# glmanhtu/vit-ed

Hardware: AMD Instinct MI355X
Metric: patch-pairs/sec fwd+bwd, div2k_erosion7_4bin_patch8_64 ViT-ED (higher is better)
Workload: dtype bf16

## Files before the change

vit-ed_amd/csrc/gemm_kernels.h:

```cpp
#pragma once
#include "gemm_epilogue.h"

int gemm_portable(const void* A, int64_t lda, const void* B, int64_t ldb, int b_layout, int dtype, int64_t M, int64_t N,
                  int64_t K, int epilogue, const EpiParams& ep, hipStream_t s);
int gemm_tn_portable(const void* dY, int64_t lddy, const void* X, int64_t ldx, int dtype, int64_t M, int64_t N, int64_t K,
                     int64_t splits, float* out, hipStream_t s);

bool gemm_nt_mfma_supported(const void* A, int64_t lda, const void* B, int64_t ldb, int64_t M, int64_t N, int64_t K,
                            int epilogue, const EpiParams& ep);
int gemm_nt_mfma(const void* A, int64_t lda, const void* B, int64_t ldb, int64_t M, int64_t N, int64_t K, int epilogue,
                 const EpiParams& ep, hipStream_t s);
bool gemm_tn_mfma_supported(const void* dY, int64_t lddy, const void* X, int64_t ldx, int64_t M, int64_t N, int64_t K);
int64_t gemm_tn_mfma_splits(int64_t M, int64_t N, int64_t K);
int gemm_tn_mfma(const void* dY, int64_t lddy, const void* X, int64_t ldx, int64_t M, int64_t N, int64_t K, int64_t splits,
                 float* out, float* bias_out , hipStream_t s);

bool gemm_tn_batch_supported(int count, const int64_t* M, const int64_t* N, const int64_t* K);
void gemm_tn_batch_layout(int count, const int64_t* M, const int64_t* N, const int64_t* K, int64_t* splits, int64_t* slab_stride,
                          int64_t* bias_stride);
int gemm_tn_batch(int count, const void* const* dY, const int64_t* lddy, const void* const* X, const int64_t* ldx, const int64_t* M,
                  const int64_t* N, const int64_t* K, const int* has_bias, float* slabs, float* bias_slabs, hipStream_t s);
int sum_slabs_batch(int count, const float* slabs, int64_t slab_stride, const float* bias_slabs, int64_t bias_stride, int64_t splits,
                    const int64_t* widths, float* const* dW, const int64_t* nbias, float* const* dbias, int accumulate, hipStream_t s);

int sum_rows_f32_single_pass(const float* in, int64_t in_ld, float* out, int64_t batch, int64_t width, hipStream_t s,
                             int accumulate = 0);
int sum_slabs_pair(const float* in_a, int64_t ld_a, float* out_a, int64_t width_a, const float* in_b, int64_t ld_b, float* out_b,
                   int64_t width_b, int64_t batch, hipStream_t s, int accumulate);
```

vit-ed_amd/csrc/gemm_mfma.hip:

```cpp
#include <stdlib.h>

#include <mutex>

#include "gemm_kernels.h"
#include "gemm_nt_epilogue.h"
#include "gemm_lds.h"

template <int BKT, int WM, bool ASM_DMA = false>
__device__ __forceinline__ void nt_stage_load(const bf16* __restrict__ A, int64_t lda, const bf16* __restrict__ B,
                                              int64_t ldb, int64_t m0, int64_t n0, int64_t M, int64_t N, int64_t k0,
                                              char* stage, int wave, int lane) {
    using C = NtCfg<BKT, WM>;
    const int rsub = lane / C::CHUNKS, cp = lane % C::CHUNKS;
#pragma unroll
    for (int i = 0; i < 32 / C::ROWS_PER_DMA; ++i) {
        const int r = wave * 32 + i * C::ROWS_PER_DMA + rsub;
        const int c = cp ^ C::swz(r);
        int64_t gm = m0 + r;
        gm = gm < M ? gm : M - 1;
        const bf16* asrc = A + gm * lda + k0 + c * 8;
        if constexpr (ASM_DMA) glds16_asm(asrc, stage + (wave * 32 + i * C::ROWS_PER_DMA) * C::ROW_BYTES);
        else glds16(asrc, stage + (wave * 32 + i * C::ROWS_PER_DMA) * C::ROW_BYTES);
    }
    constexpr int RB = BN / (2 * WM);
#pragma unroll
    for (int i = 0; i < RB / C::ROWS_PER_DMA; ++i) {
        const int r = wave * RB + i * C::ROWS_PER_DMA + rsub;
        const int c = cp ^ C::swz(r);
        int64_t gn = n0 + r;
        gn = gn < N ? gn : N - 1;
        const bf16* bsrc = B + gn * ldb + k0 + c * 8;
        if constexpr (ASM_DMA) glds16_asm(bsrc, stage + C::A_BYTES + (wave * RB + i * C::ROWS_PER_DMA) * C::ROW_BYTES);
        else glds16(bsrc, stage + C::A_BYTES + (wave * RB + i * C::ROWS_PER_DMA) * C::ROW_BYTES);
    }
}

#ifdef NT_TIMELINE
__device__ unsigned long long nt_timeline[16384 * 4];
extern "C" int vited_debug_timeline(void* dst, int64_t bytes) {
    return hipMemcpyFromSymbol(dst, HIP_SYMBOL(nt_timeline), bytes, 0, hipMemcpyDeviceToHost) == hipSuccess ? 0 : 3;
}
#endif

template <int EPI, int BKT, int WM, int STAGES = 2>
__global__ void __launch_bounds__(128 * WM)
gemm_nt_mfma_kernel(const bf16* __restrict__ A, int64_t lda, const bf16* __restrict__ B, int64_t ldb, int64_t M, int64_t N,
                    int64_t K, int tiles_n, int ntiles, EpiParams ep) {
    extern __shared__ __attribute__((aligned(16))) char smem[];
    const int lane = threadIdx.x & 63;
    const int wave = __builtin_amdgcn_readfirstlane(threadIdx.x >> 6);
    const int wr = wave >> 1, wc = wave & 1;
    const int tile = xcd_remap(blockIdx.x, ntiles);
    const int64_t m0 = (int64_t)(tile / tiles_n) * (64 * WM), n0 = (int64_t)(tile % tiles_n) * BN;

#ifdef NT_STAGGER_US
    if (blockIdx.x < 256 * NT_STAGGER_SLOTS) {
        const int slot = blockIdx.x >> 8;
        for (int i = 0; i < slot * NT_STAGGER_US; ++i) __builtin_amdgcn_s_sleep(32);
    }
#endif
#ifdef NT_TIMELINE
    const unsigned long long tl0 = __builtin_amdgcn_s_memrealtime();
#endif
    f32x4 acc[4][4];
#pragma unroll
    for (int i = 0; i < 4; ++i)
#pragma unroll
        for (int j = 0; j < 4; ++j) acc[i][j] = f32x4{0.f, 0.f, 0.f, 0.f};

    using C = NtCfg<BKT, WM>;
    constexpr bool RING = STAGES >= 3;
    constexpr int PER = 32 / C::ROWS_PER_DMA + (BN / (2 * WM)) / C::ROWS_PER_DMA;
    const int nk = (int)(K / BKT);
    nt_stage_load<BKT, WM, RING>(A, lda, B, ldb, m0, n0, M, N, 0, smem, wave, lane);
    if constexpr (RING) {
#pragma unroll
        for (int pre = 1; pre < STAGES - 1; ++pre)
            if (pre < nk) nt_stage_load<BKT, WM, RING>(A, lda, B, ldb, m0, n0, M, N, (int64_t)pre * BKT, smem + pre * C::STAGE_BYTES, wave, lane);
    }
    const int fr = lane & 15, fq = lane >> 4;
    const int64_t mtile = m0 + wr * 64, ntile = n0 + wc * 64;
    EpiPrefetch<EPI> pf;
    for (int t = 0; t < nk; ++t) {
        if constexpr (RING) {
            const int ahead = nk - 1 - t;
            if (ahead >= STAGES - 2) asm volatile("s_waitcnt vmcnt(%0) lgkmcnt(0)" ::"n"((STAGES - 2) * PER) : "memory");
            else if (ahead == 4 && STAGES > 6) asm volatile("s_waitcnt vmcnt(%0) lgkmcnt(0)" ::"n"(4 * PER) : "memory");
            else if (ahead == 3 && STAGES > 5) asm volatile("s_waitcnt vmcnt(%0) lgkmcnt(0)" ::"n"(3 * PER) : "memory");
            else if (ahead == 2 && STAGES > 4) asm volatile("s_waitcnt vmcnt(%0) lgkmcnt(0)" ::"n"(2 * PER) : "memory");
            else if (ahead == 1 && STAGES > 3) asm volatile("s_waitcnt vmcnt(%0) lgkmcnt(0)" ::"n"(PER) : "memory");
            else asm volatile("s_waitcnt vmcnt(0) lgkmcnt(0)" ::: "memory");
            __builtin_amdgcn_s_barrier();
            asm volatile("" ::: "memory");
        } else {
            asm volatile("s_waitcnt vmcnt(0)" ::: "memory");
            __syncthreads();
        }
        if (t + STAGES - 1 < nk)
            nt_stage_load<BKT, WM, RING>(A, lda, B, ldb, m0, n0, M, N, (int64_t)(t + STAGES - 1) * BKT,
                                         smem + ((t + STAGES - 1) % STAGES) * C::STAGE_BYTES, wave, lane);
        const char* sa = smem + (t % STAGES) * C::STAGE_BYTES;
        const char* sb = sa + C::A_BYTES;
        bf16x8 af[BKT / 32][4], bf_[BKT / 32][4];
#pragma unroll
        for (int kk = 0; kk < BKT / 32; ++kk) {
#pragma unroll
            for (int i = 0; i < 4; ++i) af[kk][i] = *(const bf16x8*)(sa + C::off(wr * 64 + i * 16 + fr, kk * 4 + fq));
#pragma unroll
            for (int j = 0; j < 4; ++j) bf_[kk][j] = *(const bf16x8*)(sb + C::off(wc * 64 + j * 16 + fr, kk * 4 + fq));
        }
        if constexpr (BKT == 64) __builtin_amdgcn_sched_barrier(0);
#pragma unroll
        for (int kk = 0; kk < BKT / 32; ++kk) {
#pragma unroll
            for (int i = 0; i < 4; ++i)
#pragma unroll
                for (int j = 0; j < 4; ++j) {
#ifdef NT_DBG_NO_MFMA
                    asm volatile("" ::"v"(af[kk][i]), "v"(bf_[kk][j]));
#else
                    acc[i][j] = __builtin_amdgcn_mfma_f32_16x16x32_bf16(af[kk][i], bf_[kk][j], acc[i][j], 0, 0, 0);
#endif
                }
        }
    }
#ifdef NT_DBG_NO_EPI
#pragma unroll
    for (int i = 0; i < 4; ++i)
#pragma unroll
        for (int j = 0; j < 4; ++j) asm volatile("" ::"v"(acc[i][j]));
    return;
#endif
#ifdef NT_TIMELINE
    const unsigned long long tl1 = __builtin_amdgcn_s_memrealtime();
#endif
    epilogue_prefetch_bias<EPI>(ep, pf, ntile, N, lane);
    epilogue_prefetch_subtile<EPI>(ep, pf, 0, mtile, ntile, M, N, lane);
    __syncthreads();
    float* sc = (float*)(smem + wave * SCRATCH_BYTES);
#pragma unroll
    for (int i = 0; i < 4; ++i) {
        if (i + 1 < 4) epilogue_prefetch_subtile<EPI>(ep, pf, i + 1, mtile, ntile, M, N, lane);
#pragma unroll
        for (int j = 0; j < 4; ++j)
#pragma unroll
            for (int e = 0; e < 4; ++e) sc[(fq * 4 + e) * SCRATCH_LD + j * 16 + fr] = acc[i][j][e];
        asm volatile("" ::: "memory");
        epilogue_subtile<EPI>(ep, pf, sc, i, mtile, ntile, M, N, lane);
        asm volatile("" ::: "memory");
    }
#ifdef NT_TIMELINE
    if (threadIdx.x == 0 && blockIdx.x < 16384) {
        asm volatile("s_waitcnt vmcnt(0)" ::: "memory");
        const unsigned long long tl2 = __builtin_amdgcn_s_memrealtime();
        const unsigned hw = __builtin_amdgcn_s_getreg(63492), xcc = __builtin_amdgcn_s_getreg(6164);
        nt_timeline[blockIdx.x * 4 + 0] = tl0;
        nt_timeline[blockIdx.x * 4 + 1] = tl1;
        nt_timeline[blockIdx.x * 4 + 2] = tl2;
        nt_timeline[blockIdx.x * 4 + 3] = ((unsigned long long)xcc << 32) | hw;
    }
#endif
}

bool gemm_nt_mfma_supported(const void* A, int64_t lda, const void* B, int64_t ldb, int64_t M, int64_t N, int64_t K,
                            int epilogue, const EpiParams& ep) {
    auto al16 = [](const void* p) { return ((uintptr_t)p & 15) == 0; };
    if (K % 64 || N % 16 || lda % 8 || ldb % 8 || ep.ldo % 8) return false;
    if (!al16(A) || !al16(B) || !al16(ep.out)) return false;
    if (ep.bias && !al16(ep.bias)) return false;
    if ((epilogue == VITED_EPI_GELU || epilogue == VITED_EPI_GELU_GRAD) && !al16(ep.out2)) return false;
    if ((epilogue == VITED_EPI_MUL_GELU_GRAD || epilogue == VITED_EPI_MUL) && !al16(ep.aux)) return false;
    if (epilogue == VITED_EPI_RESIDUAL && !al16(ep.residual)) return false;
    if (ceil_div64(M, 128) * ceil_div64(N, BN) > (1 << 30)) return false;
    if (M >= ((int64_t)1 << 31) || ep.rows_per_batch >= ((int64_t)1 << 31)) return false;
    return true;
}

template <int EPI, int BKT, int WM, int STAGES = 2>
static int launch_nt(const bf16* a, int64_t lda, const bf16* b, int64_t ldb, int64_t M, int64_t N, int64_t K, const EpiParams& ep,
                      hipStream_t s) {
    using C = NtCfg<BKT, WM>;
    const int tiles_n = (int)ceil_div64(N, BN);
    const int ntiles = (int)ceil_div64(M, C::BM) * tiles_n;
    auto kernel = gemm_nt_mfma_kernel<EPI, BKT, WM, STAGES>;
    constexpr int LDS = STAGES * C::STAGE_BYTES;
    if (LDS > 65536) {
        static std::once_flag once;
        static hipError_t status = hipSuccess;
        std::call_once(once, [&] { status = hipFuncSetAttribute((const void*)kernel, hipFuncAttributeMaxDynamicSharedMemorySize, LDS); });
        if (status != hipSuccess) return VITED_ERR_LAUNCH;
    }
    hipLaunchKernelGGL(kernel, dim3(ntiles), dim3(128 * WM), LDS, s, a, lda, b, ldb, M, N, K, tiles_n, ntiles, ep);
    return VITED_OK;
}

template <int EPI>
static int dispatch_nt(const bf16* a, int64_t lda, const bf16* b, int64_t ldb, int64_t M, int64_t N, int64_t K, const EpiParams& ep,
                       hipStream_t s) {
    bool shallow = K <= 512 && N >= 768;
    constexpr bool tall_epi = EPI == VITED_EPI_STORE || EPI == VITED_EPI_MUL || EPI == VITED_EPI_GELU_GRAD;
    bool tall = tall_epi && shallow && N >= 768 && M >= 8192;
#ifdef VITED_TUNING
    static const int force_bk = getenv("VITED_NT_BK") ? atoi(getenv("VITED_NT_BK")) : 0;
    static const int force_wm = getenv("VITED_NT_WM") ? atoi(getenv("VITED_NT_WM")) : 0;
    static const int force_st = getenv("VITED_NT_STAGES") ? atoi(getenv("VITED_NT_STAGES")) : 0;
    if (force_bk) shallow = force_bk == 32;
    if (force_wm) tall = force_wm == 4;
    if (force_st == 3) {
        if (shallow && tall) return launch_nt<EPI, 32, 4, 3>(a, lda, b, ldb, M, N, K, ep, s);
        if (shallow) return launch_nt<EPI, 32, 2, 3>(a, lda, b, ldb, M, N, K, ep, s);
        if (tall) return launch_nt<EPI, 64, 4, 3>(a, lda, b, ldb, M, N, K, ep, s);
        return launch_nt<EPI, 64, 2, 3>(a, lda, b, ldb, M, N, K, ep, s);
    }
#endif
    if (shallow && tall && EPI == VITED_EPI_STORE) return launch_nt<EPI, 32, 4, 3>(a, lda, b, ldb, M, N, K, ep, s);
    if (shallow && tall) return launch_nt<EPI, 32, 4>(a, lda, b, ldb, M, N, K, ep, s);
    if (shallow) return launch_nt<EPI, 32, 2>(a, lda, b, ldb, M, N, K, ep, s);
    if (tall) return launch_nt<EPI, 64, 4>(a, lda, b, ldb, M, N, K, ep, s);
    return launch_nt<EPI, 64, 2>(a, lda, b, ldb, M, N, K, ep, s);
}

int gemm_nt_mfma(const void* A, int64_t lda, const void* B, int64_t ldb, int64_t M, int64_t N, int64_t K, int epilogue,
                 const EpiParams& ep, hipStream_t s) {
    const bf16* a = (const bf16*)A;
    const bf16* b = (const bf16*)B;
    int rc;
    switch (epilogue) {
        case VITED_EPI_STORE: rc = dispatch_nt<VITED_EPI_STORE>(a, lda, b, ldb, M, N, K, ep, s); break;
        case VITED_EPI_GELU: rc = dispatch_nt<VITED_EPI_GELU>(a, lda, b, ldb, M, N, K, ep, s); break;
        case VITED_EPI_RESIDUAL: rc = dispatch_nt<VITED_EPI_RESIDUAL>(a, lda, b, ldb, M, N, K, ep, s); break;
        case VITED_EPI_MUL_GELU_GRAD: rc = dispatch_nt<VITED_EPI_MUL_GELU_GRAD>(a, lda, b, ldb, M, N, K, ep, s); break;
        case VITED_EPI_STORE_F32: rc = dispatch_nt<VITED_EPI_STORE_F32>(a, lda, b, ldb, M, N, K, ep, s); break;
        case VITED_EPI_MUL: rc = dispatch_nt<VITED_EPI_MUL>(a, lda, b, ldb, M, N, K, ep, s); break;
        case VITED_EPI_GELU_GRAD: rc = dispatch_nt<VITED_EPI_GELU_GRAD>(a, lda, b, ldb, M, N, K, ep, s); break;
        default: return VITED_ERR_BAD_ARG;
    }
    return rc != VITED_OK ? rc : vited_check_launch();
}

#ifndef TN_FORCE_TM
#define TN_FORCE_TM 0
#define TN_FORCE_STAGES 0
#endif

__device__ __forceinline__ int tn_f(int r) { return ((r & 3) << 2) | ((r >> 2) & 3); }

__device__ __forceinline__ bf16x4 tr_read(const char* p) {
    return __builtin_amdgcn_ds_read_tr16_b64_v4bf16((__attribute__((address_space(3))) bf16x4*)p);
}

template <int TM, bool ASM_DMA>
__device__ __forceinline__ void tn_stage_load(const bf16* __restrict__ dY, int64_t lddy, const bf16* __restrict__ X,
                                              int64_t ldx, int64_t mrow0, int64_t mlast, int64_t n0, int64_t N,
                                              int64_t kc0, int64_t K, char* stage, int wave, int lane) {
    constexpr int T_TILE_BYTES = TM * 128 * 2;
    const int rsub = lane >> 4, cp = lane & 15;
#pragma unroll
    for (int i = 0; i < TM / 16; ++i) {
        const int r = wave * (TM / 4) + i * 4 + rsub;
        const int ch = cp ^ tn_f(r);
        int64_t gm = mrow0 + r;
        gm = gm <= mlast ? gm : mlast;
        int64_t cn = n0 + ch * 8;
        cn = cn <= N - 8 ? cn : N - 8;
        int64_t ck = kc0 + ch * 8;
        ck = ck <= K - 8 ? ck : K - 8;
        if constexpr (ASM_DMA) {
            glds16_asm(dY + gm * lddy + cn, stage + (wave * (TM / 4) + i * 4) * 256);
            glds16_asm(X + gm * ldx + ck, stage + T_TILE_BYTES + (wave * (TM / 4) + i * 4) * 256);
        } else {
            glds16(dY + gm * lddy + cn, stage + (wave * (TM / 4) + i * 4) * 256);
            glds16(X + gm * ldx + ck, stage + T_TILE_BYTES + (wave * (TM / 4) + i * 4) * 256);
        }
    }
}

template <bool BIAS, int TM, int TN_STAGES>
__global__ void __launch_bounds__(256) __attribute__((amdgpu_waves_per_eu(3)))
gemm_tn_mfma_kernel(const bf16* __restrict__ dY, int64_t lddy, const bf16* __restrict__ X, int64_t ldx, int64_t M, int64_t N,
                    int64_t K, int64_t rows_per_split, int tiles_k, float* __restrict__ out, float* __restrict__ bias_out) {
    extern __shared__ __attribute__((aligned(16))) char smem[];
    constexpr int T_TILE_BYTES = TM * 128 * 2, T_STAGE_BYTES = 2 * T_TILE_BYTES;
    constexpr bool RING = TN_STAGES >= 3;
    const int lane = threadIdx.x & 63;
    const int wave = __builtin_amdgcn_readfirstlane(threadIdx.x >> 6);
    const int wr = wave >> 1, wc = wave & 1;
    const int ntile = gridDim.x;
    const int lin = xcd_remap(blockIdx.x + blockIdx.y * ntile, ntile * gridDim.y);
    const int split = lin / ntile, tile_id = lin - split * ntile;
    const int64_t n0 = (int64_t)(tile_id / tiles_k) * 128, kc0 = (int64_t)(tile_id % tiles_k) * 128;
    const int64_t mb = (int64_t)split * rows_per_split;
    int64_t me = mb + rows_per_split;
    me = me < M ? me : M;

    f32x4 acc[4][4];
    float bsum[4] = {0.f, 0.f, 0.f, 0.f};
#pragma unroll
    for (int i = 0; i < 4; ++i) {
#pragma unroll
        for (int j = 0; j < 4; ++j) acc[i][j] = f32x4{0.f, 0.f, 0.f, 0.f};
    }

    const int nsteps = me > mb ? (int)((me - mb + TM - 1) / TM) : 0;
    if (nsteps > 0) tn_stage_load<TM, RING>(dY, lddy, X, ldx, mb, me - 1, n0, N, kc0, K, smem, wave, lane);
    if constexpr (RING) {
#pragma unroll
        for (int pre = 1; pre < TN_STAGES - 1; ++pre)
            if (nsteps > pre) tn_stage_load<TM, RING>(dY, lddy, X, ldx, mb + pre * TM, me - 1, n0, N, kc0, K, smem + pre * T_STAGE_BYTES, wave, lane);
    }
    const int g = lane >> 4, q = (lane & 15) >> 2, p = lane & 3;
    for (int t = 0; t < nsteps; ++t) {
        if constexpr (RING) {
            constexpr int PER = 2 * (TM / 16);
            const int ahead = nsteps - 1 - t;
            if (ahead >= TN_STAGES - 2) asm volatile("s_waitcnt vmcnt(%0)" ::"n"((TN_STAGES - 2) * PER) : "memory");
            else if (ahead == 2 && TN_STAGES > 4) asm volatile("s_waitcnt vmcnt(%0)" ::"n"(2 * PER) : "memory");
            else if (ahead == 1 && TN_STAGES > 3) asm volatile("s_waitcnt vmcnt(%0)" ::"n"(PER) : "memory");
            else asm volatile("s_waitcnt vmcnt(0)" ::: "memory");
        } else {
            asm volatile("s_waitcnt vmcnt(0)" ::: "memory");
        }
        char* st = smem + (t % TN_STAGES) * T_STAGE_BYTES;
        const int64_t mrow0 = mb + (int64_t)t * TM;
        if (mrow0 + TM > me) {
            const int rsub = lane >> 4, cp = lane & 15;
#pragma unroll
            for (int i = 0; i < TM / 16; ++i) {
                const int r = wave * (TM / 4) + i * 4 + rsub;
                if (mrow0 + r >= me) {
                    *(f32x4*)(st + r * 256 + cp * 16) = f32x4{0.f, 0.f, 0.f, 0.f};
                    *(f32x4*)(st + T_TILE_BYTES + r * 256 + cp * 16) = f32x4{0.f, 0.f, 0.f, 0.f};
                }
            }
        }
        if constexpr (RING) {
            asm volatile("s_waitcnt lgkmcnt(0)" ::: "memory");
            __builtin_amdgcn_s_barrier();
            asm volatile("" ::: "memory");
        } else {
            __syncthreads();
        }
        if (t + TN_STAGES - 1 < nsteps)
            tn_stage_load<TM, RING>(dY, lddy, X, ldx, mrow0 + (TN_STAGES - 1) * TM, me - 1, n0, N, kc0, K,
                                    smem + ((t + TN_STAGES - 1) % TN_STAGES) * T_STAGE_BYTES, wave, lane);
        const char* sy = st;
        const char* sx = st + T_TILE_BYTES;
#ifdef TN_DBG_DMA_ONLY
        continue;
#endif
#pragma unroll
        for (int ms = 0; ms < TM / 32; ++ms) {
            bf16x8 af[4], bf_[4];
            const int r_lo = ms * 32 + 8 * g + q, r_hi = r_lo + 4;
            const int f_lo = tn_f(r_lo), f_hi = tn_f(r_hi);
#pragma unroll
            for (int i = 0; i < 4; ++i) {
                const int ch = ((wr * 64 + i * 16) >> 3) + (p >> 1);
                const bf16x4 lo = tr_read(sy + r_lo * 256 + ((ch ^ f_lo) << 4) + 8 * (p & 1));
                const bf16x4 hi = tr_read(sy + r_hi * 256 + ((ch ^ f_hi) << 4) + 8 * (p & 1));
                af[i] = bf16x8{lo[0], lo[1], lo[2], lo[3], hi[0], hi[1], hi[2], hi[3]};
            }
#pragma unroll
            for (int j = 0; j < 4; ++j) {
                const int ch = ((wc * 64 + j * 16) >> 3) + (p >> 1);
                const bf16x4 lo = tr_read(sx + r_lo * 256 + ((ch ^ f_lo) << 4) + 8 * (p & 1));
                const bf16x4 hi = tr_read(sx + r_hi * 256 + ((ch ^ f_hi) << 4) + 8 * (p & 1));
                bf_[j] = bf16x8{lo[0], lo[1], lo[2], lo[3], hi[0], hi[1], hi[2], hi[3]};
            }
#pragma unroll
            for (int i = 0; i < 4; ++i)
#pragma unroll
                for (int j = 0; j < 4; ++j) {
#ifdef TN_DBG_NO_MFMA
                    asm volatile("" ::"v"(af[i]), "v"(bf_[j]));
#else
                    acc[i][j] = __builtin_amdgcn_mfma_f32_16x16x32_bf16(bf_[j], af[i], acc[i][j], 0, 0, 0);
#endif
                }
            if (BIAS && kc0 == 0) {
                typedef __attribute__((ext_vector_type(2))) __bf16 bf16x2_t;
                const bf16x2_t one2 = {(__bf16)1.0f, (__bf16)1.0f};
#pragma unroll
                for (int i = 0; i < 4; ++i) {
#pragma unroll
                    for (int e = 0; e < 4; ++e)
                        bsum[i] = __builtin_amdgcn_fdot2_f32_bf16(bf16x2_t{af[i][2 * e], af[i][2 * e + 1]}, one2, bsum[i], false);
                }
            }
        }
    }
    float* o = out + (int64_t)split * N * K;
    const int fr = lane & 15, fq = lane >> 4;
#pragma unroll
    for (int i = 0; i < 4; ++i) {
#pragma unroll
        for (int j = 0; j < 4; ++j) {
            const int64_t n = n0 + wr * 64 + i * 16 + fr;
            const int64_t k = kc0 + wc * 64 + j * 16 + fq * 4;
#ifdef TN_DBG_NO_STORE
            asm volatile("" ::"v"(acc[i][j]));
#else
            if (n < N && k < K) *(f32x4*)(o + n * K + k) = acc[i][j];
#endif
        }
    }
    if constexpr (BIAS) {
        if (kc0 == 0 && wc == 0) {
            float* bo = bias_out + (int64_t)split * N;
#pragma unroll
            for (int i = 0; i < 4; ++i) {
                float v = bsum[i];
                v += __shfl_xor(v, 16);
                v += __shfl_xor(v, 32);
                const int64_t n = n0 + wr * 64 + i * 16 + fr;
                if (fq == 0 && n < N) bo[n] = v;
            }
        }
    }
}

#define TW_STAGES 4
#define TW_PANEL_BYTES (32 * 256)
#define TW_STAGE_BYTES (4 * TW_PANEL_BYTES)
#define TW_PER 4

__device__ __forceinline__ void tw_stage_issue(const bf16* const (&src)[4], char* stage, int panel, int rbase) {
#pragma unroll
    for (int i = 0; i < 4; ++i) glds16_asm(src[i], stage + panel * TW_PANEL_BYTES + (rbase + i * 4) * 256);
}

struct TwFrags {
    bf16x8 a[4], b[6];
};

__device__ __forceinline__ void tw_read_frags(TwFrags& f, const char* st, const int (&ya_lo)[4], const int (&ya_hi)[4],
                                              const int (&xb_lo)[6], const int (&xb_hi)[6]) {
#pragma unroll
    for (int i = 0; i < 4; ++i) {
        const bf16x4 lo = tr_read(st + ya_lo[i]);
        const bf16x4 hi = tr_read(st + ya_hi[i]);
        f.a[i] = bf16x8{lo[0], lo[1], lo[2], lo[3], hi[0], hi[1], hi[2], hi[3]};
    }
#pragma unroll
    for (int j = 0; j < 6; ++j) {
        const bf16x4 lo = tr_read(st + xb_lo[j]);
        const bf16x4 hi = tr_read(st + xb_hi[j]);
        f.b[j] = bf16x8{lo[0], lo[1], lo[2], lo[3], hi[0], hi[1], hi[2], hi[3]};
    }
}

#define TW_MAX_PROBLEMS 40
struct TwProblem {
    const bf16* dY;
    const bf16* X;
    int64_t lddy, ldx, M, rows_per_split;
    int64_t slab_off, bias_off;
    int N, K, tiles_k, tile0;
    int has_bias, pad_;
};
struct TwBatch {
    TwProblem p[TW_MAX_PROBLEMS];
    int64_t slab_stride, bias_stride;
    int count, total_tiles;
};

template <bool BIAS>
__global__ void __launch_bounds__(512)
gemm_tn_wide_kernel(const TwBatch batch, float* __restrict__ out_base, float* __restrict__ bias_base) {
    extern __shared__ __attribute__((aligned(16))) char smem[];
    const int lane = threadIdx.x & 63;
    const int wave = __builtin_amdgcn_readfirstlane(threadIdx.x >> 6);
    const int wr = wave >> 2, wc = wave & 3;
    const int ntile = batch.total_tiles;
    const int lin = xcd_remap(blockIdx.x + blockIdx.y * ntile, ntile * gridDim.y);
    const int split = lin / ntile;
    int tile_id = lin - split * ntile;
    int pi = 0;
    for (int i = 1; i < batch.count; ++i)
        if (batch.p[i].tile0 <= tile_id) pi = i;
    const TwProblem& pr = batch.p[pi];
    tile_id -= pr.tile0;
    const bf16* __restrict__ dY = pr.dY;
    const bf16* __restrict__ X = pr.X;
    const int64_t lddy = pr.lddy, ldx = pr.ldx, M = pr.M, N = pr.N, K = pr.K, rows_per_split = pr.rows_per_split;
    const int tiles_k = pr.tiles_k;
    const bool with_bias = BIAS && pr.has_bias;
    float* __restrict__ out = out_base + pr.slab_off;
    float* __restrict__ bias_out = bias_base + pr.bias_off;
    const int64_t n0 = (int64_t)(tile_id / tiles_k) * 128, kc0 = (int64_t)(tile_id % tiles_k) * 384;
    const int64_t mb = (int64_t)split * rows_per_split;
    int64_t me = mb + rows_per_split;
    me = me < M ? me : M;
    const int nsteps = me > mb ? (int)((me - mb + 31) / 32) : 0;

    f32x4 acc[4][6];
    float bsum[4] = {0.f, 0.f, 0.f, 0.f};
#pragma unroll
    for (int i = 0; i < 4; ++i) {
#pragma unroll
        for (int j = 0; j < 6; ++j) acc[i][j] = f32x4{0.f, 0.f, 0.f, 0.f};
    }

    const int panel = wave >> 1, rbase = (wave & 1) * 16;
    const int rsub = lane >> 4, cp = lane & 15;
    const bf16* const pbase = panel == 0 ? dY : X;
    const int64_t ld = panel == 0 ? lddy : ldx;
    const int64_t col0 = panel == 0 ? n0 : kc0 + (panel - 1) * 128;
    const int64_t colmax = panel == 0 ? N - 8 : col0 + 120;
    int64_t coff[4];
#pragma unroll
    for (int i = 0; i < 4; ++i) {
        int64_t c = col0 + ((cp ^ tn_f(rbase + i * 4 + rsub)) << 3);
        coff[i] = c <= colmax ? c : colmax;
    }
    const bf16* p0[4];
#pragma unroll
    for (int i = 0; i < 4; ++i) p0[i] = pbase + (mb + rbase + i * 4 + rsub) * ld + coff[i];
    const int64_t stage_stride = 32 * ld;
    const int rows_here = (int)(me - mb);
    auto issue = [&](int stage_idx) {
        char* dst = smem + (stage_idx & (TW_STAGES - 1)) * TW_STAGE_BYTES;
        if ((stage_idx + 1) * 32 <= rows_here) {
            const int64_t adv = (int64_t)stage_idx * stage_stride;
            const bf16* src[4];
#pragma unroll
            for (int i = 0; i < 4; ++i) src[i] = p0[i] + adv;
            tw_stage_issue(src, dst, panel, rbase);
        } else {
            const bf16* src[4];
#pragma unroll
            for (int i = 0; i < 4; ++i) {
                int r = stage_idx * 32 + rbase + i * 4 + rsub;
                r = r < rows_here ? r : rows_here - 1;
                src[i] = pbase + (mb + r) * ld + coff[i];
            }
            tw_stage_issue(src, dst, panel, rbase);
        }
    };
    auto wait_landed = [&](int idx) {
        const int later = (nsteps - 1 < idx + TW_STAGES - 2 ? nsteps - 1 : idx + TW_STAGES - 2) - idx;
        if (later >= 3 && TW_STAGES > 4) asm volatile("s_waitcnt vmcnt(%0)" ::"n"(3 * TW_PER) : "memory");
        else if (later >= 2) asm volatile("s_waitcnt vmcnt(%0)" ::"n"(2 * TW_PER) : "memory");
        else if (later == 1) asm volatile("s_waitcnt vmcnt(%0)" ::"n"(TW_PER) : "memory");
        else asm volatile("s_waitcnt vmcnt(0)" ::: "memory");
        if ((idx + 1) * 32 > rows_here) {
            char* st = smem + (idx & (TW_STAGES - 1)) * TW_STAGE_BYTES;
#pragma unroll
            for (int i = 0; i < 4; ++i) {
                const int r = rbase + i * 4 + rsub;
                if (idx * 32 + r >= rows_here) *(f32x4*)(st + panel * TW_PANEL_BYTES + r * 256 + cp * 16) = f32x4{0.f, 0.f, 0.f, 0.f};
            }
        }
    };

    const int g = lane >> 4, q = (lane & 15) >> 2, p = lane & 3;
    const int r_lo = 8 * g + q, r_hi = r_lo + 4;
    const int f_lo = tn_f(r_lo), f_hi = tn_f(r_hi);
    int ya_lo[4], ya_hi[4], xb_lo[6], xb_hi[6];
#pragma unroll
    for (int i = 0; i < 4; ++i) {
        const int ch = ((wr * 64 + i * 16) >> 3) + (p >> 1);
        ya_lo[i] = r_lo * 256 + ((ch ^ f_lo) << 4) + 8 * (p & 1);
        ya_hi[i] = r_hi * 256 + ((ch ^ f_hi) << 4) + 8 * (p & 1);
    }
#pragma unroll
    for (int j = 0; j < 6; ++j) {
        const int col = wc * 96 + j * 16;
        const int ch = ((col & 127) >> 3) + (p >> 1);
        const int base = (1 + (col >> 7)) * TW_PANEL_BYTES;
        xb_lo[j] = base + r_lo * 256 + ((ch ^ f_lo) << 4) + 8 * (p & 1);
        xb_hi[j] = base + r_hi * 256 + ((ch ^ f_hi) << 4) + 8 * (p & 1);
    }

    auto slot_l = [&](int t, TwFrags& f) {
#ifndef TW_DBG_NO_READS
        tw_read_frags(f, smem + (t & (TW_STAGES - 1)) * TW_STAGE_BYTES, ya_lo, ya_hi, xb_lo, xb_hi);
#endif
#ifndef TW_DBG_NO_DMA
        if (t + TW_STAGES - 1 < nsteps) issue(t + TW_STAGES - 1);
#endif
        __builtin_amdgcn_s_waitcnt(0xc07f);
    };
    auto slot_m = [&](const TwFrags& cur) {
        __builtin_amdgcn_s_setprio(1);
#pragma unroll
        for (int j = 0; j < 6; ++j)
#pragma unroll
            for (int i = 0; i < 4; ++i) {
#ifdef TW_DBG_NO_MFMA
                asm volatile("" ::"v"(cur.b[j]), "v"(cur.a[i]));
#else
                acc[i][j] = __builtin_amdgcn_mfma_f32_16x16x32_bf16(cur.b[j], cur.a[i], acc[i][j], 0, 0, 0);
#endif
            }
        __builtin_amdgcn_s_setprio(0);
        if (with_bias && kc0 == 0) {
            typedef __attribute__((ext_vector_type(2))) __bf16 bf16x2_t;
            const bf16x2_t one2 = {(__bf16)1.0f, (__bf16)1.0f};
#pragma unroll
            for (int i = 0; i < 4; ++i) {
#pragma unroll
                for (int e = 0; e < 4; ++e)
                    bsum[i] = __builtin_amdgcn_fdot2_f32_bf16(bf16x2_t{cur.a[i][2 * e], cur.a[i][2 * e + 1]}, one2, bsum[i], false);
            }
        }
    };
    auto barrier = [&]() {
        __builtin_amdgcn_s_barrier();
        asm volatile("" ::: "memory");
    };
    auto certify_barrier = [&](int idx) {
        __builtin_amdgcn_sched_barrier(0);
        if (idx < nsteps) {
            wait_landed(idx);
            asm volatile("s_waitcnt lgkmcnt(0)" ::: "memory");
        }
        barrier();
    };

    if (nsteps > 0) {
#pragma unroll
        for (int pre = 0; pre < TW_STAGES - 1; ++pre)
            if (nsteps > pre) issue(pre);
        certify_barrier(0);
        TwFrags f;
        if (wr == 0) {
            for (int t = 0; t < nsteps; ++t) {
                slot_l(t, f);
                barrier();
                slot_m(f);
                certify_barrier(t + 1);
            }
            barrier();
        } else {
            barrier();
            for (int t = 0; t < nsteps; ++t) {
                slot_l(t, f);
                certify_barrier(t + 1);
                slot_m(f);
                barrier();
            }
        }
    }

    float* o = out + (int64_t)split * batch.slab_stride;
    const int fr = lane & 15, fq = lane >> 4;
#pragma unroll
    for (int i = 0; i < 4; ++i) {
        const int64_t n = n0 + wr * 64 + i * 16 + fr;
#pragma unroll
        for (int j = 0; j < 6; ++j) {
            const int64_t k = kc0 + wc * 96 + j * 16 + fq * 4;
            if (n < N) *(f32x4*)(o + n * K + k) = acc[i][j];
        }
    }
    if constexpr (BIAS) {
        if (with_bias && kc0 == 0 && wc == 0) {
            float* bo = bias_out + (int64_t)split * batch.bias_stride;
#pragma unroll
            for (int i = 0; i < 4; ++i) {
                float v = bsum[i];
                v += __shfl_xor(v, 16);
                v += __shfl_xor(v, 32);
                const int64_t n = n0 + wr * 64 + i * 16 + fr;
                if (fq == 0 && n < N) bo[n] = v;
            }
        }
    }
}

bool gemm_tn_mfma_supported(const void* dY, int64_t lddy, const void* X, int64_t ldx, int64_t M, int64_t N, int64_t K) {
    auto al16 = [](const void* p) { return ((uintptr_t)p & 15) == 0; };
    return N % 8 == 0 && K % 8 == 0 && N >= 8 && K >= 8 && lddy % 8 == 0 && ldx % 8 == 0 && al16(dY) && al16(X) && M >= 1;
}

static inline bool tn_use_ring(int64_t M, int64_t N, int64_t K) {
    if (TN_FORCE_TM) return TN_FORCE_STAGES >= 3;
#ifdef VITED_TUNING
    static const char* env = getenv("VITED_TN_RING");
    if (env) return atoi(env) != 0;
#endif
    return N * K >= 1536 * 384 && M >= 16384;
}

static inline bool tn_use_wide(int64_t M, int64_t N, int64_t K) {
    if (TN_FORCE_TM) return false;
    if (K % 384 != 0) return false;
#ifdef VITED_TUNING
    static const char* env = getenv("VITED_TN_WIDE");
    if (env) return atoi(env) != 0;
#endif
    return M >= 4096;
}

int64_t gemm_tn_mfma_splits(int64_t M, int64_t N, int64_t K) {
    if (tn_use_wide(M, N, K)) {
        const int64_t tiles = ceil_div64(N, 128) * (K / 384);
        int64_t slots = 256;
#ifdef VITED_TUNING
        static const int64_t slots_env = getenv("VITED_TN_WIDE_SLOTS") ? atoi(getenv("VITED_TN_WIDE_SLOTS")) : 0;
        if (slots_env) slots = slots_env;
#endif
        int64_t s = slots / tiles;
        const int64_t max_s = ceil_div64(M, 256);
        if (s > max_s) s = max_s;
        if (s < 1) s = 1;
        const int64_t rps = ceil_div64(ceil_div64(M, s), 32) * 32;
        return ceil_div64(M, rps);
    }
    const bool ring = tn_use_ring(M, N, K);
    const int tm = TN_FORCE_TM ? TN_FORCE_TM : (ring ? 32 : 64);
    const int64_t tiles = ceil_div64(N, 128) * ceil_div64(K, 128);
    int64_t slots = tm == 64 ? 512 : 768;
#ifdef VITED_TUNING
    static const int64_t slots_env = getenv("VITED_TN_SLOTS") ? atoi(getenv("VITED_TN_SLOTS")) : 0;
    if (slots_env) slots = slots_env;
#endif
    int64_t s = slots / tiles;
    const int64_t max_s = ceil_div64(M, 512);
    if (s > max_s) s = max_s;
    if (s < 1) s = 1;
    const int64_t rps = ceil_div64(ceil_div64(M, s), tm) * tm;
    return ceil_div64(M, rps);
}

template <int TM, int STAGES>
static int launch_tn(const void* dY, int64_t lddy, const void* X, int64_t ldx, int64_t M, int64_t N, int64_t K, int64_t splits,
                      float* out, float* bias_out, hipStream_t s) {
    constexpr int LDS = STAGES * 2 * TM * 128 * 2;
    const int tiles_k = (int)ceil_div64(K, 128);
    const int tiles = (int)ceil_div64(N, 128) * tiles_k;
    const int64_t rps = ceil_div64(ceil_div64(M, splits), TM) * TM;
    if (LDS > 65536) {
        static std::once_flag once;
        static hipError_t status = hipSuccess;
        std::call_once(once, [&] {
            status = hipFuncSetAttribute((const void*)gemm_tn_mfma_kernel<true, TM, STAGES>, hipFuncAttributeMaxDynamicSharedMemorySize, LDS);
            if (status == hipSuccess)
                status = hipFuncSetAttribute((const void*)gemm_tn_mfma_kernel<false, TM, STAGES>, hipFuncAttributeMaxDynamicSharedMemorySize, LDS);
        });
        if (status != hipSuccess) return VITED_ERR_LAUNCH;
    }
    if (bias_out)
        hipLaunchKernelGGL((gemm_tn_mfma_kernel<true, TM, STAGES>), dim3(tiles, (unsigned)splits), dim3(256), LDS, s,
                           (const bf16*)dY, lddy, (const bf16*)X, ldx, M, N, K, rps, tiles_k, out, bias_out);
    else
        hipLaunchKernelGGL((gemm_tn_mfma_kernel<false, TM, STAGES>), dim3(tiles, (unsigned)splits), dim3(256), LDS, s,
                           (const bf16*)dY, lddy, (const bf16*)X, ldx, M, N, K, rps, tiles_k, out, bias_out);
    return VITED_OK;
}

static int launch_tn_wide_batch(const TwBatch& b, int64_t splits, bool any_bias, float* out, float* bias_out, hipStream_t s) {
    constexpr int LDS = TW_STAGES * TW_STAGE_BYTES;
    static std::once_flag once;
    static hipError_t status = hipSuccess;
    std::call_once(once, [&] {
        status = hipFuncSetAttribute((const void*)gemm_tn_wide_kernel<true>, hipFuncAttributeMaxDynamicSharedMemorySize, LDS);
        if (status == hipSuccess)
            status = hipFuncSetAttribute((const void*)gemm_tn_wide_kernel<false>, hipFuncAttributeMaxDynamicSharedMemorySize, LDS);
    });
    if (status != hipSuccess) return VITED_ERR_LAUNCH;
    if (any_bias)
        hipLaunchKernelGGL((gemm_tn_wide_kernel<true>), dim3(b.total_tiles, (unsigned)splits), dim3(512), LDS, s, b, out, bias_out);
    else
        hipLaunchKernelGGL((gemm_tn_wide_kernel<false>), dim3(b.total_tiles, (unsigned)splits), dim3(512), LDS, s, b, out, bias_out);
    return VITED_OK;
}

static int launch_tn_wide(const void* dY, int64_t lddy, const void* X, int64_t ldx, int64_t M, int64_t N, int64_t K, int64_t splits,
                          float* out, float* bias_out, hipStream_t s) {
    TwBatch b = {};
    TwProblem& p = b.p[0];
    p.dY = (const bf16*)dY; p.X = (const bf16*)X; p.lddy = lddy; p.ldx = ldx; p.M = M;
    p.rows_per_split = ceil_div64(ceil_div64(M, splits), 32) * 32;
    p.N = (int)N; p.K = (int)K; p.tiles_k = (int)(K / 384); p.tile0 = 0; p.has_bias = bias_out != nullptr;
    b.count = 1;
    b.total_tiles = (int)ceil_div64(N, 128) * p.tiles_k;
    b.slab_stride = N * K;
    b.bias_stride = N;
    return launch_tn_wide_batch(b, splits, bias_out != nullptr, out, bias_out, s);
}

bool gemm_tn_batch_supported(int count, const int64_t* M, const int64_t* N, const int64_t* K) {
    if (count < 1 || count > TW_MAX_PROBLEMS) return false;
    for (int i = 0; i < count; ++i)
        if (!tn_use_wide(M[i], N[i], K[i]) || N[i] % 8 || N[i] > (1 << 20) || K[i] > (1 << 20)) return false;
    return true;
}

static inline int64_t tn_batch_splits(int count, const int64_t* M, const int64_t* N, const int64_t* K) {
    int64_t tiles = 0, mmin = M[0];
    for (int i = 0; i < count; ++i) {
        tiles += ceil_div64(N[i], 128) * (K[i] / 384);
        mmin = M[i] < mmin ? M[i] : mmin;
    }
    int64_t s = 256 / tiles;
    const int64_t max_s = ceil_div64(mmin, 256);
    if (s > max_s) s = max_s;
    return s < 1 ? 1 : s;
}

void gemm_tn_batch_layout(int count, const int64_t* M, const int64_t* N, const int64_t* K, int64_t* splits, int64_t* slab_stride,
                          int64_t* bias_stride) {
    *splits = tn_batch_splits(count, M, N, K);
    int64_t w = 0, b = 0;
    for (int i = 0; i < count; ++i) {
        w += N[i] * K[i];
        b += N[i];
    }
    *slab_stride = w;
    *bias_stride = b;
}

int gemm_tn_batch(int count, const void* const* dY, const int64_t* lddy, const void* const* X, const int64_t* ldx, const int64_t* M,
                  const int64_t* N, const int64_t* K, const int* has_bias, float* slabs, float* bias_slabs, hipStream_t s) {
    TwBatch b = {};
    int64_t splits;
    gemm_tn_batch_layout(count, M, N, K, &splits, &b.slab_stride, &b.bias_stride);
    int tile = 0;
    int64_t woff = 0, boff = 0;
    bool any_bias = false;
    for (int i = 0; i < count; ++i) {
        TwProblem& p = b.p[i];
        if (!gemm_tn_mfma_supported(dY[i], lddy[i], X[i], ldx[i], M[i], N[i], K[i])) return VITED_ERR_UNSUPPORTED;
        p.dY = (const bf16*)dY[i]; p.X = (const bf16*)X[i]; p.lddy = lddy[i]; p.ldx = ldx[i]; p.M = M[i];
        p.rows_per_split = ceil_div64(ceil_div64(M[i], splits), 32) * 32;
        p.N = (int)N[i]; p.K = (int)K[i]; p.tiles_k = (int)(K[i] / 384); p.tile0 = tile; p.has_bias = has_bias[i];
        p.slab_off = woff; p.bias_off = boff;
        tile += (int)ceil_div64(N[i], 128) * p.tiles_k;
        woff += N[i] * K[i];
        boff += N[i];
        any_bias = any_bias || has_bias[i];
    }
    b.count = count;
    b.total_tiles = tile;
    const int rc = launch_tn_wide_batch(b, splits, any_bias, slabs, bias_slabs, s);
    return rc != VITED_OK ? rc : vited_check_launch();
}

int gemm_tn_mfma(const void* dY, int64_t lddy, const void* X, int64_t ldx, int64_t M, int64_t N, int64_t K, int64_t splits,
                 float* out, float* bias_out, hipStream_t s) {
    int rc;
    if (tn_use_wide(M, N, K)) rc = launch_tn_wide(dY, lddy, X, ldx, M, N, K, splits, out, bias_out, s);
#if TN_FORCE_TM
    else rc = launch_tn<TN_FORCE_TM, TN_FORCE_STAGES>(dY, lddy, X, ldx, M, N, K, splits, out, bias_out, s);
#else
    else if (tn_use_ring(M, N, K)) rc = launch_tn<32, 3>(dY, lddy, X, ldx, M, N, K, splits, out, bias_out, s);
    else rc = launch_tn<64, 2>(dY, lddy, X, ldx, M, N, K, splits, out, bias_out, s);
#endif
    return rc != VITED_OK ? rc : vited_check_launch();
}
```

Before: 42510.

## Add persistent register-resident-A NT GEMM kernel for K=384 shapes

Adds a persistent GEMM kernel for K=384. Each wave keeps its full A panel (32 rows by 384) in registers and streams 128-column weight tiles through a multi-slot LDS ring with async global-to-LDS loads, walking across N tiles before advancing panels. It is dispatched by default for the EPI_MUL epilogue (8 waves, aux operand staged in LDS) and for EPI_STORE with N>=1152 and M>=65536 (4 waves). The aim is to stop re-fetching A per output tile and to overlap weight loads with MFMA work. In exchange it adds heavy register pressure, hand-counted vmcnt waits that are fragile, and a new code path for these shapes.

Result: faster. 43560, median of 6 (+2.5%).

```diff
diff --git a/profiles/nt_k384_probe.py b/profiles/nt_k384_probe.py
--- /dev/null
+++ b/profiles/nt_k384_probe.py
@@ -0,0 +1,74 @@
+#!/usr/bin/env python3
+import argparse
+import json
+import os
+import statistics
+import sys
+
+import torch
+
+sys.path.insert(0, os.path.dirname(os.path.dirname(os.path.abspath(__file__))))
+import vited_amd as v
+
+ops, L = v.ops, v._lib
+
+SHAPES = [('qkv', 1152, L.EPI_STORE), ('kv', 768, L.EPI_STORE), ("fc1+gelu'", 1536, L.EPI_GELU_GRAD), ("dz=dy.W2*gelu'", 1536, L.EPI_MUL)]
+K = 384
+
+
+def main():
+    ap = argparse.ArgumentParser()
+    ap.add_argument('--rows', type=int, nargs='+', default=[65536, 66560, 24576, 73800])
+    ap.add_argument('--rounds', type=int, default=7)
+    ap.add_argument('--reps', type=int, default=50)
+    ap.add_argument('--modes', type=int, nargs='+', default=[0, 8, 4])
+    ap.add_argument('--json', default=None)
+    a = ap.parse_args()
+    dev = torch.device('cuda:0')
+    g = torch.Generator(device='cpu').manual_seed(0)
+
+    def rnd(*shape, scale=1.0):
+        return (torch.randn(*shape, generator=g) * scale).to(dev)
+
+    results = []
+    for M in a.rows:
+        print(f'M = {M}   (us per launch: median [min .. max] over {a.rounds} rounds of {a.reps})')
+        for name, n, epi in SHAPES:
+            x, w = rnd(M, K).bfloat16(), rnd(n, K, scale=0.05).bfloat16()
+            kw = dict(epilogue=epi)
+            if epi == L.EPI_MUL:
+                kw['aux'] = rnd(M, n).bfloat16()
+            else:
+                kw['bias'] = rnd(n)
+            kw['out'] = torch.empty(M, n, device=dev, dtype=torch.bfloat16)
+            if epi == L.EPI_GELU_GRAD:
+                kw['out2'] = torch.empty(M, n, device=dev, dtype=torch.bfloat16)
+            times = {m: [] for m in a.modes}
+            for m in a.modes:
+                os.environ['VITED_NT_AREG'] = str(m)
+                for _ in range(3):
+                    ops.gemm(x, w, **kw)
+            torch.cuda.synchronize()
+            for _ in range(a.rounds):
+                for m in a.modes:
+                    os.environ['VITED_NT_AREG'] = str(m)
+                    e0, e1 = torch.cuda.Event(enable_timing=True), torch.cuda.Event(enable_timing=True)
+                    e0.record()
+                    for _ in range(a.reps):
+                        ops.gemm(x, w, **kw)
+                    e1.record()
+                    torch.cuda.synchronize()
+                    times[m].append(e0.elapsed_time(e1) / a.reps * 1e3)
+            line = f'  {name:16s} N={n:5d}'
+            for m in a.modes:
+                t = times[m]
+                line += f' | mode {m}: {statistics.median(t):7.1f} [{min(t):7.1f} .. {max(t):7.1f}]'
+                results.append(dict(M=M, shape=name, N=n, mode=m, us=t))
+            print(line, flush=True)
+    if a.json:
+        with open(a.json, 'w') as f:
+            json.dump(results, f)
+
+
+if __name__ == '__main__':
+    main()
diff --git a/vit-ed_amd/csrc/gemm_kernels.h b/vit-ed_amd/csrc/gemm_kernels.h
--- a/vit-ed_amd/csrc/gemm_kernels.h
+++ b/vit-ed_amd/csrc/gemm_kernels.h
@@ -9,6 +9,9 @@
 bool gemm_nt_mfma_supported(const void* A, int64_t lda, const void* B, int64_t ldb, int64_t M, int64_t N, int64_t K,
                             int epilogue, const EpiParams& ep);
 int gemm_nt_mfma(const void* A, int64_t lda, const void* B, int64_t ldb, int64_t M, int64_t N, int64_t K, int epilogue,
+                 const EpiParams& ep, hipStream_t s);
+bool gemm_nt_areg_supported(int64_t ldw, int64_t M, int64_t N, int64_t K, int epilogue);
+int gemm_nt_areg(const void* A, int64_t lda, const void* W, int64_t ldw, int64_t M, int64_t N, int epilogue, int waves,
                  const EpiParams& ep, hipStream_t s);
 bool gemm_tn_mfma_supported(const void* dY, int64_t lddy, const void* X, int64_t ldx, int64_t M, int64_t N, int64_t K);
 int64_t gemm_tn_mfma_splits(int64_t M, int64_t N, int64_t K);
diff --git a/vit-ed_amd/csrc/gemm_mfma.hip b/vit-ed_amd/csrc/gemm_mfma.hip
--- a/vit-ed_amd/csrc/gemm_mfma.hip
+++ b/vit-ed_amd/csrc/gemm_mfma.hip
@@ -12,6 +12,7 @@
                                               char* stage, int wave, int lane) {
     using C = NtCfg<BKT, WM>;
     const int rsub = lane / C::CHUNKS, cp = lane % C::CHUNKS;
+#ifndef NT_DBG_NO_A_DMA
 #pragma unroll
     for (int i = 0; i < 32 / C::ROWS_PER_DMA; ++i) {
         const int r = wave * 32 + i * C::ROWS_PER_DMA + rsub;
@@ -22,6 +23,7 @@
         if constexpr (ASM_DMA) glds16_asm(asrc, stage + (wave * 32 + i * C::ROWS_PER_DMA) * C::ROW_BYTES);
         else glds16(asrc, stage + (wave * 32 + i * C::ROWS_PER_DMA) * C::ROW_BYTES);
     }
+#endif
     constexpr int RB = BN / (2 * WM);
 #pragma unroll
     for (int i = 0; i < RB / C::ROWS_PER_DMA; ++i) {
@@ -70,7 +72,11 @@
 
     using C = NtCfg<BKT, WM>;
     constexpr bool RING = STAGES >= 3;
+#ifdef NT_DBG_NO_A_DMA
+    constexpr int PER = (BN / (2 * WM)) / C::ROWS_PER_DMA;
+#else
     constexpr int PER = 32 / C::ROWS_PER_DMA + (BN / (2 * WM)) / C::ROWS_PER_DMA;
+#endif
     const int nk = (int)(K / BKT);
     nt_stage_load<BKT, WM, RING>(A, lda, B, ldb, m0, n0, M, N, 0, smem, wave, lane);
     if constexpr (RING) {
@@ -194,9 +200,20 @@
     return VITED_OK;
 }
 
+template <int EPI> static inline int nt_areg_waves(int64_t ldb, int64_t M, int64_t N, int64_t K) {
+    if (!gemm_nt_areg_supported(ldb, M, N, K, EPI)) return 0;
+#ifdef VITED_TUNING
+    if (const char* force = getenv("VITED_NT_AREG")) return atoi(force);
+#endif
+    if (EPI == VITED_EPI_MUL) return 8;
+    if (EPI == VITED_EPI_STORE && N >= 1152 && M >= 65536) return 4;
+    return 0;
+}
+
 template <int EPI>
 static int dispatch_nt(const bf16* a, int64_t lda, const bf16* b, int64_t ldb, int64_t M, int64_t N, int64_t K, const EpiParams& ep,
                        hipStream_t s) {
+    if (const int waves = nt_areg_waves<EPI>(ldb, M, N, K)) return gemm_nt_areg(a, lda, b, ldb, M, N, EPI, waves, ep, s);
     bool shallow = K <= 512 && N >= 768;
     constexpr bool tall_epi = EPI == VITED_EPI_STORE || EPI == VITED_EPI_MUL || EPI == VITED_EPI_GELU_GRAD;
     bool tall = tall_epi && shallow && N >= 768 && M >= 8192;
diff --git a/vit-ed_amd/csrc/gemm_nt_k384.hip b/vit-ed_amd/csrc/gemm_nt_k384.hip
--- /dev/null
+++ b/vit-ed_amd/csrc/gemm_nt_k384.hip
@@ -0,0 +1,245 @@
+#include <mutex>
+#include <type_traits>
+
+#include "gemm_kernels.h"
+#include "gemm_nt_epilogue.h"
+#include "gemm_lds.h"
+
+#define NT_AREG_CHUNK_BYTES (128 * 128)
+#define NT_AREG_KSTEPS 12
+#define NT_AREG_MAX_N 2048
+
+static constexpr __host__ __device__ int nt_areg_slots(int waves, int epi) { return waves == 8 && epi != VITED_EPI_MUL ? 6 : 3; }
+static constexpr __host__ __device__ bool nt_areg_aux_lds(int waves, int epi) { return waves == 8 && epi == VITED_EPI_MUL; }
+#define NT_AREG_AUX_BYTES (32 * 128 * 2)
+static constexpr __host__ __device__ int nt_areg_lds_bytes(int waves, int epi) {
+    return nt_areg_slots(waves, epi) * NT_AREG_CHUNK_BYTES + waves * SCRATCH_BYTES + NT_AREG_MAX_N * 4 +
+           (nt_areg_aux_lds(waves, epi) ? waves * NT_AREG_AUX_BYTES : 0);
+}
+
+template <int EPI, int WAVES>
+__global__ void __launch_bounds__(64 * WAVES) __attribute__((amdgpu_waves_per_eu(2, 2)))
+gemm_nt_areg_kernel(const bf16* __restrict__ A, int64_t lda, const bf16* __restrict__ W, int64_t ldw, int64_t M, int64_t N,
+                    int tiles_n, int nitems, EpiParams ep) {
+    extern __shared__ __attribute__((aligned(16))) char smem[];
+    using C = NtCfg<64>;
+    constexpr int PM = 32 * WAVES;
+    constexpr int PER = 16 / WAVES;
+    constexpr int S = nt_areg_slots(WAVES, EPI), D = S - 1;
+    constexpr bool AUX_LDS = nt_areg_aux_lds(WAVES, EPI);
+    static_assert(!AUX_LDS || D < 6, "a chunk issued behind the multiplier rows must be waited for before the epilogue");
+    constexpr int E = EPI == VITED_EPI_STORE || AUX_LDS ? 8 : 16;
+    const int lane = threadIdx.x & 63;
+    const int wave = __builtin_amdgcn_readfirstlane(threadIdx.x >> 6);
+    const int fr = lane & 15, fq = lane >> 4;
+
+    const int share = xcd_remap(blockIdx.x, gridDim.x);
+    const int begin = (int)((int64_t)share * nitems / gridDim.x), end = (int)((int64_t)(share + 1) * nitems / gridDim.x);
+    if (begin >= end) return;
+
+    unsigned woff[PER];
+#pragma unroll
+    for (int j = 0; j < PER; ++j) {
+        const int r = (wave * PER + j) * 8 + (lane >> 3);
+        woff[j] = (unsigned)r * (unsigned)ldw + (unsigned)(((lane & 7) ^ C::swz(r)) << 3);
+    }
+    auto issue = [&](int nt, int kc) {
+        const bf16* base = W + (int64_t)nt * 128 * ldw + kc * 64;
+        char* dst = smem + (kc % S) * NT_AREG_CHUNK_BYTES + wave * PER * 1024;
+#pragma unroll
+        for (int j = 0; j < PER; ++j) glds16_asm(base + woff[j], dst + j * 1024);
+    };
+    int boff[2];
+#pragma unroll
+    for (int kk = 0; kk < 2; ++kk) boff[kk] = C::off(fr, kk * 4 + fq);
+    float* sc = (float*)(smem + S * NT_AREG_CHUNK_BYTES + wave * SCRATCH_BYTES);
+    float* sbias = (float*)(smem + S * NT_AREG_CHUNK_BYTES + WAVES * SCRATCH_BYTES);
+    for (int n = threadIdx.x; n < (int)N; n += 64 * WAVES) sbias[n] = ep.bias ? ep.bias[n] : 0.f;
+    char* saux = smem + S * NT_AREG_CHUNK_BYTES + WAVES * SCRATCH_BYTES + NT_AREG_MAX_N * 4 + wave * NT_AREG_AUX_BYTES;
+
+    auto issue_aux = [&](int panel_, int nt_) {
+        const int64_t mt_ = (int64_t)panel_ * PM + wave * 32, n0_ = (int64_t)nt_ * 128;
+#pragma unroll
+        for (int s = 0; s < 4; ++s)
+#pragma unroll
+            for (int pc = 0; pc < 2; ++pc) {
+                int64_t m = mt_ + (s & 1) * 16 + pc * 8 + (lane >> 3);
+                m = m < M ? m : M - 1;
+                glds16_asm((const bf16*)ep.aux + m * ep.ldo + n0_ + (s >> 1) * 64 + (lane & 7) * 8, saux + (s * 2 + pc) * 1024);
+            }
+    };
+    int panel = begin / tiles_n, nt = begin - panel * tiles_n;
+    int loaded = -1;
+    bf16x8 a[2][NT_AREG_KSTEPS];
+#pragma unroll
+    for (int kc = 0; kc < D; ++kc) issue(nt, kc);
+    if constexpr (AUX_LDS) issue_aux(panel, nt);
+    bool prev_full = false;
+    for (int it = begin; it < end; ++it) {
+        if (panel != loaded) {
+#pragma unroll
+            for (int i = 0; i < 2; ++i) {
+                int64_t gm = (int64_t)panel * PM + wave * 32 + i * 16 + fr;
+                gm = gm < M ? gm : M - 1;
+                const bf16* arow = A + gm * lda + fq * 8;
+#pragma unroll
+                for (int ks = 0; ks < NT_AREG_KSTEPS; ++ks) a[i][ks] = *(const bf16x8*)(arow + ks * 32);
+            }
+            __builtin_amdgcn_s_waitcnt(0x0f70);
+            loaded = panel;
+        }
+        int next_nt = nt + 1, next_panel = panel;
+        if (next_nt == tiles_n) {
+            next_nt = 0;
+            ++next_panel;
+        }
+        const bool has_next = it + 1 < end;
+
+        const int64_t mt = (int64_t)panel * PM + wave * 32, n0 = (int64_t)nt * 128;
+        const bool full = mt + 32 <= M;
+        const bool counted = prev_full && full;
+        EpiPrefetch<EPI> pf[2];
+        if constexpr (EPI == VITED_EPI_MUL && !AUX_LDS) epilogue_prefetch_subtile<EPI>(ep, pf[0], 0, mt, n0, M, N, lane);
+        f32x4 acc[2][8];
+#pragma unroll
+        for (int i = 0; i < 2; ++i)
+#pragma unroll
+            for (int j = 0; j < 8; ++j) acc[i][j] = f32x4{0.f, 0.f, 0.f, 0.f};
+
+        auto step = [&](auto kc_) {
+            constexpr int kc = decltype(kc_)::value;
+            constexpr int lo = kc < D ? 0 : kc - D + 1;
+            constexpr int before = kc < D ? D - kc - 1 : 0;
+            constexpr int n_next = before + (kc - lo);
+            constexpr int n_last = before + ((6 - D < kc ? 6 - D : kc) > lo ? (6 - D < kc ? 6 - D : kc) - lo : 0);
+            constexpr int AUXN = AUX_LDS && kc < D ? 8 : 0;
+            if (has_next) {
+                if (kc < D && counted) asm volatile("s_waitcnt vmcnt(%0) lgkmcnt(0)" ::"n"(n_next * PER + AUXN + E) : "memory");
+                else asm volatile("s_waitcnt vmcnt(%0) lgkmcnt(0)" ::"n"(n_next * PER + AUXN) : "memory");
+            } else {
+                if (kc < D && counted) asm volatile("s_waitcnt vmcnt(%0) lgkmcnt(0)" ::"n"(n_last * PER + AUXN + E) : "memory");
+                else asm volatile("s_waitcnt vmcnt(%0) lgkmcnt(0)" ::"n"(n_last * PER + AUXN) : "memory");
+            }
+            __builtin_amdgcn_s_barrier();
+            asm volatile("" ::: "memory");
+#ifndef NT_DBG_NO_W_DMA
+            if constexpr (kc + D < 6) issue(nt, kc + D);
+            else if (has_next) issue(next_nt, kc + D - 6);
+#endif
+            const char* sb = smem + (kc % S) * NT_AREG_CHUNK_BYTES;
+            bf16x8 bfr[8];
+            auto read4 = [&](int kk, int g) {
+#pragma unroll
+                for (int j = 0; j < 4; ++j) bfr[g * 4 + j] = *(const bf16x8*)(sb + (g * 4 + j) * 16 * C::ROW_BYTES + boff[kk]);
+            };
+            auto mfma8 = [&](int kk, int g) {
+#pragma unroll
+                for (int j = 0; j < 4; ++j)
+#pragma unroll
+                    for (int i = 0; i < 2; ++i)
+                        acc[i][g * 4 + j] = __builtin_amdgcn_mfma_f32_16x16x32_bf16(a[i][kc * 2 + kk], bfr[g * 4 + j], acc[i][g * 4 + j], 0, 0, 0);
+            };
+            read4(0, 0);
+            read4(0, 1);
+            __builtin_amdgcn_sched_barrier(0);
+            mfma8(0, 0);
+            __builtin_amdgcn_sched_barrier(0);
+            read4(1, 0);
+            __builtin_amdgcn_sched_barrier(0);
+            mfma8(0, 1);
+            __builtin_amdgcn_sched_barrier(0);
+            read4(1, 1);
+            __builtin_amdgcn_sched_barrier(0);
+            mfma8(1, 0);
+            mfma8(1, 1);
+        };
+        step(std::integral_constant<int, 0>{});
+        step(std::integral_constant<int, 1>{});
+        step(std::integral_constant<int, 2>{});
+        step(std::integral_constant<int, 3>{});
+        step(std::integral_constant<int, 4>{});
+        step(std::integral_constant<int, 5>{});
+
+#ifdef NT_DBG_NO_EPI
+#pragma unroll
+        for (int i = 0; i < 2; ++i)
+#pragma unroll
+            for (int j = 0; j < 8; ++j) asm volatile("" ::"v"(acc[i][j]));
+#else
+        if constexpr (AUX_LDS) {
+#pragma unroll
+            for (int s = 0; s < 4; ++s)
+#pragma unroll
+                for (int pc = 0; pc < 2; ++pc) pf[s >> 1].aux[s & 1][pc] = *(const bf16x8*)(saux + (s * 2 + pc) * 1024 + lane * 16);
+            asm volatile("s_waitcnt lgkmcnt(0)" ::: "memory");
+            if (has_next) issue_aux(next_panel, next_nt);
+        } else if constexpr (EPI == VITED_EPI_MUL) {
+            epilogue_prefetch_subtile<EPI>(ep, pf[0], 1, mt, n0, M, N, lane);
+            epilogue_prefetch_subtile<EPI>(ep, pf[1], 0, mt, n0 + 64, M, N, lane);
+            epilogue_prefetch_subtile<EPI>(ep, pf[1], 1, mt, n0 + 64, M, N, lane);
+        }
+#pragma unroll
+        for (int h = 0; h < 2; ++h) {
+            const float* bp = sbias + n0 + h * 64 + EpiTraits<EPI>::col(lane);
+            pf[h].bias[0] = *(const f32x4*)bp;
+            pf[h].bias[1] = *(const f32x4*)(bp + 4);
+        }
+#pragma unroll
+        for (int s = 0; s < 4; ++s) {
+            const int h = s >> 1, i = s & 1;
+#pragma unroll
+            for (int j = 0; j < 4; ++j)
+#pragma unroll
+                for (int e = 0; e < 4; ++e) sc[(fq * 4 + e) * SCRATCH_LD + j * 16 + fr] = acc[i][h * 4 + j][e];
+            asm volatile("" ::: "memory");
+            epilogue_subtile<EPI>(ep, pf[h], sc, i, mt, n0 + h * 64, M, N, lane);
+            asm volatile("" ::: "memory");
+        }
+#endif
+        prev_full = full;
+        panel = next_panel;
+        nt = next_nt;
+    }
+}
+
+bool gemm_nt_areg_supported(int64_t ldw, int64_t M, int64_t N, int64_t K, int epilogue) {
+    if (epilogue != VITED_EPI_STORE && epilogue != VITED_EPI_MUL && epilogue != VITED_EPI_GELU_GRAD) return false;
+    if (K != 32 * NT_AREG_KSTEPS || N % 128 || N < 768 || M < 8192) return false;
+    return ldw < (1 << 20) && N <= NT_AREG_MAX_N && ceil_div64(M, 128) * (N / 128) < (1 << 30);
+}
+
+template <int EPI, int WAVES>
+static int launch_areg(const bf16* a, int64_t lda, const bf16* w, int64_t ldw, int64_t M, int64_t N, const EpiParams& ep, hipStream_t s) {
+    constexpr int LDS = nt_areg_lds_bytes(WAVES, EPI);
+    auto kernel = gemm_nt_areg_kernel<EPI, WAVES>;
+    static std::once_flag once;
+    static hipError_t status = hipSuccess;
+    std::call_once(once, [&] { status = hipFuncSetAttribute((const void*)kernel, hipFuncAttributeMaxDynamicSharedMemorySize, LDS); });
+    if (status != hipSuccess) return VITED_ERR_LAUNCH;
+    const int tiles_n = (int)(N / 128);
+    const int nitems = (int)ceil_div64(M, 32 * WAVES) * tiles_n;
+    const int slots = WAVES == 8 ? 256 : 512;
+    const int grid = nitems < slots ? nitems : slots;
+    hipLaunchKernelGGL(kernel, dim3(grid), dim3(64 * WAVES), LDS, s, a, lda, w, ldw, M, N, tiles_n, nitems, ep);
+    return VITED_OK;
+}
+
+int gemm_nt_areg(const void* A, int64_t lda, const void* W, int64_t ldw, int64_t M, int64_t N, int epilogue, int waves,
+                 const EpiParams& ep, hipStream_t s) {
+    const bf16* a = (const bf16*)A;
+    const bf16* w = (const bf16*)W;
+    if (waves != 4 && waves != 8) return VITED_ERR_BAD_ARG;
+    if (epilogue == VITED_EPI_MUL && waves == 8) return launch_areg<VITED_EPI_MUL, 8>(a, lda, w, ldw, M, N, ep, s);
+    if (epilogue == VITED_EPI_STORE && waves == 4) return launch_areg<VITED_EPI_STORE, 4>(a, lda, w, ldw, M, N, ep, s);
+#ifdef VITED_TUNING
+    switch (epilogue) {
+        case VITED_EPI_STORE: return launch_areg<VITED_EPI_STORE, 8>(a, lda, w, ldw, M, N, ep, s);
+        case VITED_EPI_MUL: return launch_areg<VITED_EPI_MUL, 4>(a, lda, w, ldw, M, N, ep, s);
+        case VITED_EPI_GELU_GRAD:
+            return waves == 8 ? launch_areg<VITED_EPI_GELU_GRAD, 8>(a, lda, w, ldw, M, N, ep, s)
+                              : launch_areg<VITED_EPI_GELU_GRAD, 4>(a, lda, w, ldw, M, N, ep, s);
+        default: break;
+    }
+#endif
+    return VITED_ERR_UNSUPPORTED;
+}
```
